# dphoyes/OpenCL-Structure-from-Motion

Measured on AMD Instinct MI355X. Metric: stereo frame-pairs/sec (1242x375) through pushBack+matchFeatures(2), p_matched bit-exact, higher is better.
Workload: dtype u8

## Files before the change

opencl-structure-from-motion_amd/csrc/vsm_dc.hip:

```cpp
#include <hip/hip_runtime.h>
#include <atomic>
#include <stdint.h>
#include <stdio.h>

#include <algorithm>
#include <mutex>
#include <vector>
#include <cmath>

#include "vsm_dc_gpu.h"
#include "vsm_dc_mesh.h"
#include "vsm_dc_lds.h"
#include "vsm_internal.h"

static const uint32_t *dc2_tiny_table();

#define KD_THREADS 1024
#define KD_CHUNKS 256
#define KD_DIGITS 128

__device__ inline uint32_t kd_block_scan(uint32_t v, uint32_t *tot) {
  const int lane = threadIdx.x & 63, wv = threadIdx.x >> 6;
  uint32_t x = v;
#pragma unroll
// ... 1224 lines not shown
      const int32_t div = nn[e] >> 1;
      if (q < off[e] + div) {
        nn[e] = div;
      } else {
        off[e] += div;
        nn[e] -= div;
      }
    }
    __syncthreads();
    if (cut_x) {
      uint16_t *w = Y;
      Y = Yn;
      Yn = w;
    } else {
      uint16_t *w = X;
      X = Xn;
      Xn = w;
    }
  }
  DC2_T(p4);
#pragma unroll
  for (int e = 0; e < E; e++) {
    const int q = E * t + e;
    if (q < m) jb.key[q] = jb.key_sorted[X[q]];
  }
#ifdef DC2_PHASE_TIMING
  if (t == 0) {
    const long long p5 = clock64();
    atomicAdd(&dc2_dbg[12][0], 1ull);
    DC2_ACC(12, 3, p2, p3);
    DC2_ACC(12, 4, p3, p4);
    DC2_ACC(12, 2, p4, p5);
  }
#endif
}

__device__ inline bool dc2_walk(int32_t m, int depth, uint32_t path, int32_t &off, int32_t &n, int &axis) {
  off = 0;
  n = m;
  axis = 0;
  for (int b = depth - 1; b >= 0; b--) {
    if (n <= VSM_DC_BLOCK_POINTS) return false;
    const int32_t div = n >> 1;
    if ((path >> b) & 1) {
      off += div;
      n -= div;
    } else {
      n = div;
    }
    axis = 1 - axis;
  }
  return true;
}

#define DC2_REACH_ALL 0x7fff8000u
#define DC2_REACH_NONE 0x80007fffu
__device__ inline uint32_t dc2_reach_word(double c, double rad) {
  const double lo = floor(c - rad), hi = ceil(c + rad);
  if (!(lo == lo) || !(hi == hi)) return DC2_REACH_ALL;
  const int32_t l = lo < -32768.0 ? -32768 : (lo > 32767.0 ? 32767 : (int32_t)lo);
  const int32_t h = hi > 32767.0 ? 32767 : (hi < -32768.0 ? -32768 : (int32_t)hi);
  return ((uint32_t)l & 0xffffu) | ((uint32_t)h << 16);
}
__device__ inline void dc2_reach(uint32_t pa, uint32_t pb, uint32_t pc, uint32_t &wx, uint32_t &wy) {
  const double ax = (double)(pa & 0xffffu), ay = (double)(pa >> 16);
  const double bx = (double)(pb & 0xffffu) - ax, by = (double)(pb >> 16) - ay;
  const double cx = (double)(pc & 0xffffu) - ax, cy = (double)(pc >> 16) - ay;
  const double d = 2.0 * (bx * cy - by * cx);
  const double b2 = bx * bx + by * by, c2 = cx * cx + cy * cy;
  const double ux = (cy * b2 - by * c2) / d, uy = (bx * c2 - cx * b2) / d;
  const double rad = sqrt(ux * ux + uy * uy) + 1.5;
  if (!(d == d) || d == 0.0 || !(rad == rad)) {
    wx = wy = DC2_REACH_ALL;
    return;
  }
  wx = dc2_reach_word(ax + ux, rad);
  wy = dc2_reach_word(ay + uy, rad);
}
__device__ inline bool dc2_reaches(uint32_t w, bool left_half, int32_t cl, int32_t cr) {
  const int32_t lo = (int32_t)(int16_t)(w & 0xffffu), hi = (int32_t)(int16_t)(w >> 16);
  return left_half ? hi >= cr : lo <= cl;
}

#ifndef DC2_BLOCK_WAVES
#define DC2_BLOCK_WAVES 4
#endif
#define DC2_BLOCK_THREADS (64 * DC2_BLOCK_WAVES)
#ifndef DC2_BLOCK_PACKED
#define DC2_BLOCK_PACKED 16
#endif
#ifndef DC2_BLOCK_OCC
#define DC2_BLOCK_OCC 5
#endif
#ifndef DC2_BLOCK_TAIL
#if defined(__gfx900__) || defined(__gfx906__) || defined(__gfx908__) || defined(__gfx90a__) || defined(__gfx940__) || defined(__gfx941__) || \
    defined(__gfx942__) || defined(__gfx950__) || !defined(__HIP_DEVICE_COMPILE__)
#define DC2_BLOCK_TAIL 1
#else
#define DC2_BLOCK_TAIL DC2_BLOCK_WAVES
#endif
#endif
__global__ void __launch_bounds__(DC2_BLOCK_THREADS, DC2_BLOCK_OCC) k_dc2_block(const VsmDc2Job *__restrict__ jobs, int depth) {
  __shared__ __attribute__((aligned(16))) uint32_t s_w[2 * VSM_DC_BLOCK_POINTS * 4];
  __shared__ uint32_t s_pt[VSM_DC_BLOCK_POINTS];
  __shared__ Dc2Hull16 s_hull[2 << DC2_BLOCK_DEPTH];
  const VsmDc2Job j2 = jobs[blockIdx.y];
  const int32_t m = j2.mn[0];
  if (m < 2) return;
  int32_t boff = 0, bn = m;
  int baxis = 0, d = 0;
  uint32_t bidx = 1;
  const uint32_t path = blockIdx.x;
  for (int b = depth - 1; b >= 0 && bn > VSM_DC_BLOCK_POINTS; b--, d++) {
    const int32_t div = bn >> 1;
    if ((path >> b) & 1) {
      boff += div;
      bn -= div;
      bidx = 2 * bidx + 1;
    } else {
      bn = div;
      bidx = 2 * bidx;
    }
    baxis = 1 - baxis;
  }
  if (bn > VSM_DC_BLOCK_POINTS) {
    if (threadIdx.x == 0) *j2.error = 2;
    return;
  }
  if (d < depth && (path & ((1u << (depth - d)) - 1u)) != 0) return;
  const int lane = threadIdx.x;
  const int wv = lane >> 6, wl = lane & 63;
  DC2_T(c0);
  {
    dc2_v4u ones;
    ones.x = ones.y = ones.z = ones.w = 0xffffffffu;
    for (int i = lane; i < 2 * bn; i += DC2_BLOCK_THREADS) ((dc2_v4u *)s_w)[i] = ones;
  }
  __syncthreads();
  DcBlockMesh mesh;
  mesh.w = (DC2_AS3 dc2_u32a *)s_w;
  mesh.pt = (DC2_AS3 const uint32_t *)s_pt;
  mesh.key = j2.key + boff;
  mesh.ptw = (DC2_AS3 uint32_t *)s_pt;
  mesh.gid = j2.id + boff;
  DC2_T(c1);
  {
    constexpr int kPerWave = (1 << DC2_BLOCK_DEPTH) / DC2_BLOCK_WAVES;
    for (int v = wl; v < kPerWave; v += 64) dc2_block_leaf_run(mesh, wv * kPerWave + v, bn, baxis, (DC2_AS3 Dc2Hull16 *)s_hull);
  }
  __syncthreads();
  DC2_T(c2);
#ifdef DC2_PHASE_TIMING
  long long cl = c2;
#endif
  for (int L = DC2_BLOCK_DEPTH - 1; L >= 0; L--) {
    {
      const int nodes = 1 << L;
      int node = -1;
      if (nodes >= DC2_BLOCK_PACKED) {
        if (DC2_BLOCK_TAIL < DC2_BLOCK_WAVES && wv >= DC2_BLOCK_TAIL && wv * 64 >= nodes) return;
        node = lane < nodes ? lane : -1;
      } else if (nodes >= DC2_BLOCK_TAIL) {
        const int per_wave = nodes / DC2_BLOCK_TAIL;
        if (wv >= DC2_BLOCK_TAIL) return;
        node = wl < per_wave ? wv * per_wave + wl : -1;
      } else {
        if (wv >= nodes && DC2_BLOCK_TAIL < DC2_BLOCK_WAVES) return;
        node = wl == 0 && wv < nodes ? wv : -1;
      }
      if (node >= 0) dc2_block_merge_run(mesh, node, L, bn, baxis, (DC2_AS3 Dc2Hull16 *)s_hull);
    }
    __syncthreads();
#ifdef DC2_PHASE_TIMING
    {
      const long long cn = clock64();
      if (lane == 0) DC2_ACC(0, 3 + L, cl, cn);
      cl = cn;
    }
#endif
  }
  DC2_T(c3);
  dc2_v4i *gt = (dc2_v4i *)(j2.tri + (size_t)2 * boff * 8);
  constexpr int kLive = DC2_BLOCK_TAIL < DC2_BLOCK_WAVES ? 64 : DC2_BLOCK_THREADS;
  for (int t = lane; t < 2 * bn; t += kLive) {
    const dc2_v4u o = ((const dc2_v4u *)s_w)[t];
    auto nb = [&](uint32_t v) -> int32_t { return (v & 0xffffu) == 0xffffu ? -1 : (int32_t)(v & 0xffffu) + 8 * boff; };
    auto vx = [&](uint32_t v) -> int32_t { return (v >> 16) == 0xffffu ? -1 : (int32_t)(v >> 16) + boff; };
    dc2_v4i a, b;
    a.x = nb(o.x);
    a.y = nb(o.y);
    a.z = nb(o.z);
    b.x = vx(o.x);
    b.y = vx(o.y);
    b.z = vx(o.z);
    uint32_t wx, wy;
    if ((b.x & b.y & b.z) < 0)
      wx = wy = DC2_REACH_NONE;
    else if ((b.x | b.y | b.z) < 0)
      wx = wy = DC2_REACH_ALL;
    else
      dc2_reach(s_pt[o.x >> 16], s_pt[o.y >> 16], s_pt[o.z >> 16], wx, wy);
    a.w = (int32_t)wy;
    b.w = (int32_t)wx;
    gt[2 * t] = a;
    gt[2 * t + 1] = b;
  }
  for (int i = lane; i < bn; i += kLive) j2.pt[boff + i] = s_pt[i];
  if (lane == 0) {
    const Dc2Hull16 hl = s_hull[1];
    j2.hulls[bidx] = VsmDcHull{hl.fl_t + 2 * boff, hl.fl_o, hl.fr_t + 2 * boff, hl.fr_o};
  }
#ifdef DC2_PHASE_TIMING
  if (lane == 0) {
    const long long c4 = clock64();
    atomicAdd(&dc2_dbg[0][0], 1ull);
    DC2_ACC(0, 1, c0, c1);
    DC2_ACC(0, 2, c1, c2);
    DC2_ACC(0, 13, c3, c4);
    DC2_ACC(0, 14, c0, c4);
  }
#endif
}

#ifndef DC2_MERGE_THREADS
#define DC2_MERGE_THREADS 256
#endif
#ifndef DC2_BAND_BATCH
#define DC2_BAND_BATCH 8
#endif
#ifdef DC2_PHASE_TIMING
#define DC2_BAND_STAT(level, col, v) atomicAdd(&dc2_dbg[1 + (level)][col], (unsigned long long)(v))
#else
#define DC2_BAND_STAT(level, col, v)
#endif

__device__ inline uint32_t dc2_mask_prefix(const uint32_t *mask, uint16_t *pre, int words, uint32_t *tot) {
  const int t = threadIdx.x, lane = t & 63, wv = t >> 6;
  const int per = (words + DC2_MERGE_THREADS - 1) / DC2_MERGE_THREADS;
  const int w0 = min(words, t * per), w1 = min(words, w0 + per);
  uint32_t sum = 0;
  for (int w = w0; w < w1; w++) sum += __popc(mask[w]);
  uint32_t x = sum;
#pragma unroll
  for (int d = 1; d < 64; d <<= 1) {
    const uint32_t y = __shfl_up(x, d, 64);
    if (lane >= d) x += y;
  }
  if (lane == 63) tot[wv] = x;
  __syncthreads();
  uint32_t base = 0, total = 0;
  for (int k = 0; k < DC2_MERGE_THREADS / 64; k++) {
    base += k < wv ? tot[k] : 0u;
    total += tot[k];
  }
  uint32_t run = base + x - sum;
  for (int w = w0; w < w1; w++) {
    pre[w] = (uint16_t)run;
    run += __popc(mask[w]);
  }
  __syncthreads();
  return total;
}
__device__ inline bool dc2_bit(const uint32_t *mask, int i) { return (mask[i >> 5] >> (i & 31)) & 1u; }
__device__ inline int dc2_rank(const uint32_t *mask, const uint16_t *pre, int i) {
  return (int)pre[i >> 5] + __popc(mask[i >> 5] & ((1u << (i & 31)) - 1u));
}

__global__ void __launch_bounds__(DC2_MERGE_THREADS) k_dc2_merge(const VsmDc2Job *__restrict__ jobs, int level, int lines_cap, int pts_cap, int words_cap) {
  extern __shared__ __attribute__((aligned(16))) uint8_t dc2_lds[];
  uint16_t *s_rec = (uint16_t *)dc2_lds;
  uint32_t *s_pt = (uint32_t *)(s_rec + (size_t)lines_cap * 8);
  uint32_t *s_l2s = s_pt + pts_cap;
  uint32_t *s_c2p = s_l2s + lines_cap;
  uint32_t *s_band = s_c2p + pts_cap;
  uint32_t *s_ring = s_band + words_cap;
  uint32_t *s_pmask = s_ring + words_cap;
  uint16_t *s_bpre = (uint16_t *)(s_pmask + (words_cap + 1) / 2);
  uint16_t *s_ppre = s_bpre + words_cap;
  __shared__ int32_t s_cl, s_cr, s_fail;
  __shared__ uint32_t s_tot[DC2_MERGE_THREADS / 64];
  const VsmDc2Job jb = jobs[blockIdx.y];
  const int32_t m = jb.mn[0];
  if (m < 2) return;
  int32_t off, n;
  int axis;
  if (!dc2_walk(m, level, blockIdx.x, off, n, axis) || n <= VSM_DC_BLOCK_POINTS) return;
  const uint32_t idx = (1u << level) | blockIdx.x;
  const int t = threadIdx.x;
  const int32_t div = n >> 1;
  const VsmDcHull l = jb.hulls[2 * idx], r = jb.hulls[2 * idx + 1];
  const int32_t tbase = 2 * off, nslots = 2 * n, tbase4 = 4 * tbase;
  const int bwords = (nslots + 31) >> 5, pwords = (n + 31) >> 5;
  int32_t *gnode = jb.tri + (size_t)tbase * 8;
  const dc2_v4i *grec = (const dc2_v4i *)gnode;
  const uint32_t *gpt = jb.pt + off;
  DC2_T(m0);
  bool band_ok = bwords <= words_cap;
  if (t == 0) {
    s_cl = -1;
    s_cr = 1 << 30;
    s_fail = 0;
  }
  if (band_ok) {
    for (int i = t; i < bwords; i += DC2_MERGE_THREADS) {
      s_band[i] = 0;
      s_ring[i] = 0;
    }
    for (int i = t; i < pwords; i += DC2_MERGE_THREADS) s_pmask[i] = 0;
    __syncthreads();
    {
      int32_t cl = -1, cr = 1 << 30;
      for (int i0 = t; i0 < n; i0 += DC2_BAND_BATCH * DC2_MERGE_THREADS) {
        uint32_t p[DC2_BAND_BATCH];
#pragma unroll
        for (int k = 0; k < DC2_BAND_BATCH; k++) {
          const int i = i0 + k * DC2_MERGE_THREADS;
          p[k] = i < n ? gpt[i] : 0u;
        }
#pragma unroll
        for (int k = 0; k < DC2_BAND_BATCH; k++) {
          const int i = i0 + k * DC2_MERGE_THREADS;
          const int32_t c = axis == 0 ? (int32_t)(p[k] & 0xffffu) : (int32_t)(p[k] >> 16);
          if (i < div)
            cl = max(cl, c);
          else if (i < n)
            cr = min(cr, c);
        }
      }
#pragma unroll
      for (int o = 32; o >= 1; o >>= 1) {
        cl = max(cl, __shfl_xor(cl, o, 64));
        cr = min(cr, __shfl_xor(cr, o, 64));
      }
      if ((t & 63) == 0) {
        atomicMax(&s_cl, cl);
        atomicMin(&s_cr, cr);
      }
    }
    __syncthreads();
    const int32_t cl = s_cl, cr = s_cr;
    {
      const int32_t *gw = gnode + (axis == 0 ? 7 : 3);
      for (int s0 = t; s0 < nslots; s0 += DC2_BAND_BATCH * DC2_MERGE_THREADS) {
        uint32_t w[DC2_BAND_BATCH];
#pragma unroll
        for (int k = 0; k < DC2_BAND_BATCH; k++) {
          const int s = s0 + k * DC2_MERGE_THREADS;
          w[k] = s < nslots ? (uint32_t)gw[(size_t)s * 8] : DC2_REACH_NONE;
        }
#pragma unroll
        for (int k = 0; k < DC2_BAND_BATCH; k++) {
          const int s = s0 + k * DC2_MERGE_THREADS;
          const bool hot = s < nslots && (s == 2 * div - 2 || s == 2 * div - 1 || dc2_reaches(w[k], s < 2 * div, cl, cr));
          if (hot) atomicOr(&s_band[s >> 5], 1u << (s & 31));
        }
      }
    }
    __syncthreads();
    const int s_own = 2 * div - 2;
    for (int s0 = t; s0 < nslots; s0 += DC2_BAND_BATCH * DC2_MERGE_THREADS) {
      dc2_v4i e[DC2_BAND_BATCH];
      bool hot[DC2_BAND_BATCH];
#pragma unroll
      for (int k = 0; k < DC2_BAND_BATCH; k++) {
        const int s = s0 + k * DC2_MERGE_THREADS;
        hot[k] = s < nslots && dc2_bit(s_band, s);
        e[k] = grec[2 * (hot[k] ? s : s_own)];
      }
#pragma unroll
      for (int k = 0; k < DC2_BAND_BATCH; k++) {
        if (!hot[k]) continue;
        const int32_t nb[3] = {e[k].x, e[k].y, e[k].z};
#pragma unroll
        for (int o = 0; o < 3; o++) {
          if (nb[o] < 0) continue;
          const int s2 = (nb[o] - tbase4) >> 2;
          if (s2 >= 0 && s2 < nslots) atomicOr(&s_ring[s2 >> 5], 1u << (s2 & 31));
        }
      }
    }
    __syncthreads();
    for (int i = t; i < bwords; i += DC2_MERGE_THREADS) s_band[i] |= s_ring[i];
    __syncthreads();
    const uint32_t nlines = dc2_mask_prefix(s_band, s_bpre, bwords, s_tot);
    uint32_t npts = 0;
    band_ok = nlines + 1 <= (uint32_t)lines_cap;
    if (band_ok) {
      for (int s = t; s < nslots; s += DC2_MERGE_THREADS)
        if (dc2_bit(s_band, s)) s_l2s[dc2_rank(s_band, s_bpre, s)] = (uint32_t)s;
      __syncthreads();
      for (uint32_t k0 = t; k0 < nlines; k0 += 3 * DC2_MERGE_THREADS) {
        dc2_v4i v[3];
#pragma unroll
        for (int k = 0; k < 3; k++) {
          const uint32_t ln = k0 + k * DC2_MERGE_THREADS;
          v[k] = grec[2 * (ln < nlines ? (int)s_l2s[ln] : s_own) + 1];
        }
#pragma unroll
        for (int k = 0; k < 3; k++) {
          if (k0 + k * DC2_MERGE_THREADS >= nlines) continue;
          const int32_t vv[3] = {v[k].x, v[k].y, v[k].z};
#pragma unroll
          for (int o = 0; o < 3; o++)
            if (vv[o] >= 0) atomicOr(&s_pmask[(vv[o] - off) >> 5], 1u << ((vv[o] - off) & 31));
        }
      }
      __syncthreads();
      npts = dc2_mask_prefix(s_pmask, s_ppre, pwords, s_tot);
      band_ok = npts <= (uint32_t)pts_cap;
      if (band_ok) {
        for (int i0 = t; i0 < n; i0 += DC2_BAND_BATCH * DC2_MERGE_THREADS) {
          uint32_t p[DC2_BAND_BATCH];
#pragma unroll
          for (int k = 0; k < DC2_BAND_BATCH; k++) {
            const int i = i0 + k * DC2_MERGE_THREADS;
            p[k] = gpt[i < n ? i : 0];
          }
#pragma unroll
          for (int k = 0; k < DC2_BAND_BATCH; k++) {
            const int i = i0 + k * DC2_MERGE_THREADS;
            if (i < n && dc2_bit(s_pmask, i)) {
              const int c = dc2_rank(s_pmask, s_ppre, i);
              s_pt[c] = p[k];
              s_c2p[c] = (uint32_t)i;
            }
          }
        }
        for (uint32_t k0 = t; k0 < nlines; k0 += 3 * DC2_MERGE_THREADS) {
          dc2_v4i e3[3], v3[3];
#pragma unroll
          for (int k = 0; k < 3; k++) {
            const uint32_t ln = k0 + k * DC2_MERGE_THREADS;
            const int s = ln < nlines ? (int)s_l2s[ln] : s_own;
            e3[k] = grec[2 * s];
            v3[k] = grec[2 * s + 1];
          }
#pragma unroll
          for (int k = 0; k < 3; k++) {
            const uint32_t line = k0 + k * DC2_MERGE_THREADS;
            if (line >= nlines) continue;
            const dc2_v4i e = e3[k], v = v3[k];
            auto nbw = [&](int32_t g) -> uint32_t {
              if (g < 0) return 4 * nlines;
              const int s2 = (g - tbase4) >> 2;
              if (s2 < 0 || s2 >= nslots || !dc2_bit(s_band, s2)) return 4 * nlines;
              return (uint32_t)(dc2_rank(s_band, s_bpre, s2) * 4 + (g & 3));
            };
            auto vxw = [&](int32_t g) -> uint32_t { return g < 0 ? 0xffffu : (uint32_t)dc2_rank(s_pmask, s_ppre, g - off); };
            dc2_v4u o;
            o.x = nbw(e.x) | (vxw(v.x) << 16);
            o.y = nbw(e.y) | (vxw(v.y) << 16);
            o.z = nbw(e.z) | (vxw(v.z) << 16);
            o.w = 0xffffffffu;
            ((dc2_v4u *)s_rec)[line] = o;
          }
        }
      }
    }
    __syncthreads();
    DC2_T(m1);
    if (band_ok) {
      if (t == 0) {
        DcBandMesh mesh;
        mesh.w = (DC2_AS3 dc2_u32a *)s_rec;
        mesh.pt = (DC2_AS3 const uint32_t *)s_pt;
        mesh.rim = 4 * (int32_t)nlines;
        mesh.budget = 8 * (int32_t)nlines + 64;
        mesh.make_trap();
        auto ln = [&](int32_t gt) -> int32_t {
          if (!dc2_bit(s_band, gt - tbase)) mesh.tripped = 1;
          return dc2_rank(s_band, s_bpre, gt - tbase);
        };
        DcOTri fl{ln(l.fl_t), l.fl_o}, il{ln(l.fr_t), l.fr_o}, ir{ln(r.fl_t), r.fl_o}, fr{ln(r.fr_t), r.fr_o};
        int32_t tcur = dc2_rank(s_band, s_bpre, 2 * div - 2);
        if (mesh.ok()) dc_merge(mesh, fl, il, ir, fr, axis, tcur);
        if (mesh.ok() && !mesh.trap_touched())
          jb.hulls[idx] = VsmDcHull{(int32_t)s_l2s[fl.t] + tbase, fl.o, (int32_t)s_l2s[fr.t] + tbase, fr.o};
        else
          s_fail = 1;
      }
      __syncthreads();
      band_ok = s_fail == 0;
#ifdef DC2_PHASE_TIMING
      if (t == 0) {
        const long long m2 = clock64();
        atomicAdd(&dc2_dbg[1 + level][0], 1ull);
        DC2_ACC(1 + level, 1, m0, m1);
        DC2_ACC(1 + level, 2, m1, m2);
        DC2_BAND_STAT(level, 3, nlines);
        DC2_BAND_STAT(level, 4, band_ok ? 0 : 1);
        atomicMax(&dc2_dbg[1 + level][6], (unsigned long long)nlines);
        atomicMax(&dc2_dbg[1 + level][7], (unsigned long long)npts);
      }
#endif
      if (band_ok) {
        for (uint32_t k = t; k < nlines; k += DC2_MERGE_THREADS) {
          const dc2_v4u o = ((const dc2_v4u *)s_rec)[k];
          auto nb = [&](uint32_t v) -> int32_t { return v == 0xffffu ? -1 : (int32_t)(s_l2s[v >> 2] * 4 + (v & 3)) + tbase4; };
          auto vx = [&](uint32_t v) -> int32_t { return v == 0xffffu ? -1 : (int32_t)s_c2p[v] + off; };
          const uint32_t rimh = 4 * nlines;
          const int32_t s = (int32_t)s_l2s[k];
          const dc2_v4i old = grec[2 * s];
          dc2_v4i a, b;
          a.x = (o.x & 0xffffu) == rimh ? old.x : nb(o.x & 0xffffu);
          a.y = (o.y & 0xffffu) == rimh ? old.y : nb(o.y & 0xffffu);
          a.z = (o.z & 0xffffu) == rimh ? old.z : nb(o.z & 0xffffu);
          b.x = vx(o.x >> 16);
          b.y = vx(o.y >> 16);
          b.z = vx(o.z >> 16);
          uint32_t wx, wy;
          if ((b.x & b.y & b.z) < 0)
            wx = wy = DC2_REACH_NONE;
          else if ((b.x | b.y | b.z) < 0)
            wx = wy = DC2_REACH_ALL;
          else
            dc2_reach(s_pt[o.x >> 16], s_pt[o.y >> 16], s_pt[o.z >> 16], wx, wy);
          a.w = (int32_t)wy;
          b.w = (int32_t)wx;
          ((dc2_v4i *)gnode)[2 * s] = a;
          ((dc2_v4i *)gnode)[2 * s + 1] = b;
        }
        return;
      }
    }
  }
  if (t == 0) {
    DcOTri fl{l.fl_t, l.fl_o}, il{l.fr_t, l.fr_o}, ir{r.fl_t, r.fl_o}, fr{r.fr_t, r.fr_o};
    int32_t tg = 2 * (off + div) - 2;
    const DcMesh mesh{jb.tri, jb.pt, jb.id, jb.key};
    mesh.merge_hulls(fl, il, ir, fr, axis, tg);
    jb.hulls[idx] = VsmDcHull{fl.t, fl.o, fr.t, fr.o};
#ifdef DC2_PHASE_TIMING
    atomicAdd(&dc2_dbg[1 + level][5], 1ull);
#endif
  }
  __threadfence();
  __syncthreads();
  for (int sl = t; sl < nslots; sl += DC2_MERGE_THREADS) {
    const int32_t vx0 = __hip_atomic_load(gnode + (size_t)sl * 8 + 4, __ATOMIC_RELAXED, __HIP_MEMORY_SCOPE_AGENT);
    const int32_t vx1 = __hip_atomic_load(gnode + (size_t)sl * 8 + 5, __ATOMIC_RELAXED, __HIP_MEMORY_SCOPE_AGENT);
    const int32_t vx2 = __hip_atomic_load(gnode + (size_t)sl * 8 + 6, __ATOMIC_RELAXED, __HIP_MEMORY_SCOPE_AGENT);
    uint32_t wx, wy;
    if ((vx0 & vx1 & vx2) < 0)
      wx = wy = DC2_REACH_NONE;
    else if ((vx0 | vx1 | vx2) < 0)
      wx = wy = DC2_REACH_ALL;
    else
      dc2_reach(jb.pt[vx0], jb.pt[vx1], jb.pt[vx2], wx, wy);
    gnode[(size_t)sl * 8 + 3] = (int32_t)wy;
    gnode[(size_t)sl * 8 + 7] = (int32_t)wx;
  }
}

template <int CAP>
__global__ void __launch_bounds__(64) k_dc2_ties(const VsmDc2Job *__restrict__ jobs, int32_t *__restrict__ tie_out, int out_stride, const uint32_t *__restrict__ tiny) {
  const VsmDc2Job jb = jobs[blockIdx.x];
  int32_t *out = tie_out ? tie_out + (size_t)blockIdx.x * out_stride : const_cast<int32_t *>(jb.tie_out);
  const int n = *jb.count;
  if (n <= 3 || n > jb.cap) {
    if (threadIdx.x == 0) out[0] = n <= 3 ? 0 : -1;
    return;
  }
  tie_sort<CAP>(TieFromKeys{jb.keys_in}, n, out, tiny);
}

__global__ void __launch_bounds__(64) k_dc2_apply_ties(const VsmDc2Job *__restrict__ jobs) {
  const VsmDc2Job jb = jobs[blockIdx.x];
  const int32_t c = jb.tie_out[0];
  if (c < 0) {
    if (threadIdx.x == 0 && jb.mn[0] >= 2) *jb.error = 3;
    return;
  }
  for (int k = threadIdx.x; k < c; k += 64) {
    const int32_t rep = jb.tie_out[1 + 2 * k], first = jb.tie_out[2 + 2 * k];
    if (rep >= 0 && rep < jb.cap) jb.remap[rep] = first;
  }
}

__global__ void __launch_bounds__(256) k_dc2_flows(const VsmDc2Job *__restrict__ jobs, int method) {
  const VsmDc2Job jb = jobs[blockIdx.y];
  const int n = jb.mn[1];
  const int i = blockIdx.x * blockDim.x + threadIdx.x;
  if (i >= n || jb.mn[0] < 2) return;
  const vsm_p_match a = jb.list[i];
  float *fu = (float *)jb.kd_scratch, *fv = fu + jb.kd_stride, *dp = fv + jb.kd_stride;
  fu[i] = a.u1c - a.u1p;
  fv[i] = a.v1c - a.v1p;
  dp[i] = method == 1 ? a.u1c - a.u2c : a.u1p - a.u2p;
}

__global__ void __launch_bounds__(256) k_dc2_support(const VsmDc2Job *__restrict__ jobs, int method, float ftol, float dtol) {
  const VsmDc2Job jb = jobs[blockIdx.y];
  const int32_t m = jb.mn[0];
  const int t = blockIdx.x * blockDim.x + threadIdx.x;
  if (m < 2 || t >= 2 * m) return;
  const int4 v = *(const int4 *)(jb.tri + (size_t)t * 8 + 4);
  if ((v.x | v.y | v.z) < 0) return;
  const int32_t q[3] = {jb.remap[jb.id[v.y]], jb.remap[jb.id[v.z]], jb.remap[jb.id[v.x]]};
  const float *fua = (const float *)jb.kd_scratch, *fva = fua + jb.kd_stride, *dpa = fva + jb.kd_stride;
  float fu[3], fv[3], dp[3];
#pragma unroll
  for (int k = 0; k < 3; k++) {
    fu[k] = fua[q[k]];
    fv[k] = fva[q[k]];
    dp[k] = dpa[q[k]];
  }
#pragma unroll
  for (int e = 0; e < 3; e++) {
// ... 334 lines not shown
```

opencl-structure-from-motion_amd/csrc/vsm_seq2.inc:

```
#include "vsm_dc_gpu.h"

struct Dc2Bank {
  int npairs = 0, cap = 0;
  bool host_ties = false;
  uint8_t *d_block = nullptr, *h_block = nullptr, *h_block_dev = nullptr;
  VsmDc2Job *h_jobs = nullptr, *d_jobs = nullptr;
  int32_t *d_ties = nullptr;
  uint64_t *h_keys = nullptr;
  int32_t *h_n = nullptr, *h_ties = nullptr, *h_error = nullptr;
  int ties_stride = 0;
  size_t pair_stride = 0;
  struct PairPtr {
    uint64_t *keys_in, *key_sorted, *key;
    uint32_t *kd, *pt;
    int32_t *id, *tri, *mn, *support, *remap, *out_count;
    VsmDcHull *hulls;
  };
  std::vector<PairPtr> pp;
  void release() {
    if (d_block) vsm_dev_free(d_block);
    if (h_block) (void)hipHostFree(h_block);
    if (h_jobs) (void)hipHostFree(h_jobs);
    *this = Dc2Bank();
  }
  static size_t al(size_t x) { return (x + 255) & ~(size_t)255; }
  bool reserve(int pairs, int want_cap, bool with_host_ties) {
    if (pairs <= npairs && want_cap <= cap && (!with_host_ties || host_ties)) return true;
    const int ncap = std::max(((want_cap + 1023) / 1024) * 1024, cap), np = std::max(pairs, npairs);
    const bool ht = with_host_ties || host_ties;
    release();
    npairs = np;
    cap = ncap;
    host_ties = ht;
    const size_t c = (size_t)cap;
    const size_t per = al(c * 8) * 3 + al(c * 4 * VSM_DC_KD_SCRATCH) + al(c * 4) * 4 + al(c * 64) + al(64) +
                       al(sizeof(VsmDcHull) * (2u << VSM_DC2_MAX_DEPTH));
    pair_stride = per;
    const size_t d_bytes = per * npairs + al(sizeof(VsmDc2Job) * npairs) + al((size_t)npairs * VSM_DC_TIE_OUT_INTS * 4);
    ties_stride = cap + 2;
    const size_t h_bytes = al(64) + (ht ? (al(c * 8) + al((size_t)ties_stride * 4)) * npairs : 0) + al((size_t)npairs * 4);
    if (vsm_dev_alloc((void **)&d_block, d_bytes) != hipSuccess || hipHostMalloc((void **)&h_block, h_bytes, hipHostMallocMapped) != hipSuccess ||
        hipHostGetDevicePointer((void **)&h_block_dev, h_block, 0) != hipSuccess ||
        hipHostMalloc((void **)&h_jobs, sizeof(VsmDc2Job) * npairs, hipHostMallocDefault) != hipSuccess) {
      release();
      return false;
    }
    memset(h_block, 0, h_bytes);
    pp.resize(npairs);
    uint8_t *b = d_block;
    auto take = [&](size_t bytes) {
      uint8_t *r = b;
      b += al(bytes);
      return r;
    };
    for (int i = 0; i < npairs; i++) {
      PairPtr &q = pp[i];
      q.keys_in = (uint64_t *)take(c * 8);
      q.key_sorted = (uint64_t *)take(c * 8);
      q.key = (uint64_t *)take(c * 8);
      q.kd = (uint32_t *)take(c * 4 * VSM_DC_KD_SCRATCH);
      q.pt = (uint32_t *)take(c * 4);
      q.id = (int32_t *)take(c * 4);
      q.support = (int32_t *)take(c * 4);
      q.remap = (int32_t *)take(c * 4);
      q.tri = (int32_t *)take(c * 64);
      q.mn = (int32_t *)take(64);
      q.out_count = q.mn + 4;
      q.hulls = (VsmDcHull *)take(sizeof(VsmDcHull) * (2u << VSM_DC2_MAX_DEPTH));
    }
    d_jobs = (VsmDc2Job *)take(sizeof(VsmDc2Job) * npairs);
    d_ties = (int32_t *)take((size_t)npairs * VSM_DC_TIE_OUT_INTS * 4);
    size_t ho = 0;
    h_error = (int32_t *)(h_block + ho);
    ho += al(64);
    h_n = (int32_t *)(h_block + ho);
    ho += al((size_t)npairs * 4);
    if (ht) {
      h_keys = (uint64_t *)(h_block + ho);
      ho += al(c * 8) * npairs;
      h_ties = (int32_t *)(h_block + ho);
    }
    return true;
  }
  uint64_t *host_keys(int i) const { return (uint64_t *)((uint8_t *)h_keys + al((size_t)cap * 8) * i); }
  int32_t *host_ties_of(int i) const { return (int32_t *)((uint8_t *)h_ties + al((size_t)ties_stride * 4) * i); }
  template <typename T>
  T *dev_of(T *host_ptr) const {
    return (T *)(h_block_dev + ((uint8_t *)host_ptr - h_block));
  }
  void fill_job(int i, const vsm_p_match *list, const int32_t *count, bool gpu_ties, vsm_p_match *out, int32_t *h_out_count,
                float *ranges, uint32_t *h_keep = nullptr, bool keys_by_dma = false) {
    const PairPtr &q = pp[i];
    VsmDc2Job &jb = h_jobs[i];
    memset(&jb, 0, sizeof(jb));
    jb.list = list;
    jb.count = count;
    jb.cap = cap;
    jb.kd_stride = cap;
    jb.keys_in = q.keys_in;
    jb.h_keys = (!gpu_ties && host_ties && !keys_by_dma) ? dev_of(host_keys(i)) : nullptr;
    jb.h_n = dev_of(h_n + i);
    jb.key_sorted = q.key_sorted;
    jb.key = q.key;
    jb.kd_scratch = q.kd;
    jb.pt = q.pt;
    jb.id = q.id;
    jb.tri = q.tri;
    jb.hulls = q.hulls;
    jb.mn = q.mn;
    jb.support = q.support;
// ... 746 lines not shown
      for (int j = 0; j < k; j++) {
        const int rc = finish_chain1_of(j);
        if (rc != VSM_OK) return rc;
      }
    const double t0 = now_us();
    HIPCHK(hipEventSynchronize(h->seq_ev[0]));
    HIPCHK(hipGetLastError());
    tg += now_us() - t0;
    dbg_counts.push_back(now_us());
    q.max_nq[0] = q.max_nq[1] = 0;
    q.valid = std::make_shared<std::vector<char>>(n, 0);
    for (int i = 0; i < n; i++) {
      const int32_t f = q.f0 + i;
      VsmJob &jb = h_jobs[i];
      memset(&jb, 0, sizeof(jb));
      const int img_c = first_img + sides * i;
      int img_p;
      int32_t cnt[4][2];
      for (int s = 0; s < 2; s++) {
        cnt[2][s] = c.hm_counts[img_c * 2 + s];
        cnt[3][s] = right ? c.hm_counts[(img_c + 1) * 2 + s] : 0;
      }
      if (method == 1) {
        img_p = img_c;
        for (int s = 0; s < 2; s++) cnt[0][s] = cnt[1][s] = 0;
      } else if (i > 0) {
        img_p = img_c - sides;
        for (int s = 0; s < 2; s++) {
          cnt[0][s] = c.hm_counts[img_p * 2 + s];
          cnt[1][s] = right ? c.hm_counts[(img_p + 1) * 2 + s] : 0;
        }
      } else {
        img_p = sides * ((k + kFrameBanks - 1) % kFrameBanks) * C + sides * ((k > 0 ? chunk_start[k] - chunk_start[k - 1] : 1) - 1);
        for (int s = 0; s < 2; s++) {
          cnt[0][s] = f > 0 ? nprev[0][s] : 0;
          cnt[1][s] = f > 0 ? nprev[1][s] : 0;
        }
      }
      jb.img_prev = img_p;
      jb.img_curr = img_c;
      if (match_ready(p, method, cnt)) {
        (*q.valid)[i] = 1;
        const int qimg = method == 2 ? 0 : 2;
        jb.nq[0] = p.multi_stage ? cnt[qimg][0] : 0;
        jb.nq[1] = cnt[qimg][1];
        if (Tr && (!Tr_valid || Tr_valid[f])) {
          jb.use_tr = 1;
          memcpy(jb.t, Tr + (size_t)f * 12, 12 * sizeof(double));
        }
      }
      q.max_nq[0] = std::max(q.max_nq[0], jb.nq[0]);
      q.max_nq[1] = std::max(q.max_nq[1], jb.nq[1]);
    }
    for (int s = 0; s < 2; s++) {
      nprev[0][s] = c.hm_counts[(first_img + sides * (n - 1)) * 2 + s];
      nprev[1][s] = right ? c.hm_counts[(first_img + sides * (n - 1) + 1) * 2 + s] : 0;
    }
    if (q.max_nq[0] > VSM_DC_TIE_POINTS || q.max_nq[1] > VSM_DC_KD_MAX_POINTS || (p.refinement == 2 && q.max_nq[1] > VSM_PARA_MAX_LIST) ||
        vsm_dc2_depth(std::max(q.max_nq[0], q.max_nq[1])) > VSM_DC2_MAX_DEPTH) {
      declined = true;
      return VSM_OK;
    }
    HIPCHK(vsm_upload(h->stream, d_jobs, h_jobs, sizeof(VsmJob) * n));
    if (p.multi_stage) {
      VsmMatchCfg cfg = make_cfg(p, method, h->sw.match_heads && c.has_heads);
      VsmJob dummy;
      memset(&dummy, 0, sizeof(dummy));
      cfg.sparse = 1;
      cfg.use_prior = 0;
      vsm_launch_match(h->stream, h->prof, c.d_imgs, d_pairs, d_jobs, dummy, n, c.dims, cfg, q.max_nq[0]);
      q.ev_p1 = S.get_event();
      q.ev_prior = S.get_event();
      if (!q.ev_p1 || !q.ev_prior) return VSM_EHIP;
      HIPCHK(hipEventRecord(q.ev_p1, h->stream));
    }
    return VSM_OK;
  };
  auto start_chain1 = [&](int k) -> int {
    Ck &q = ck[k];
    if (!p.multi_stage) return VSM_OK;
    const int n = q.n, first_pair = q.first_pair;
    {
      Dc2Bank &B = S.bank1[k & 1];
      if (!B.reserve(C, std::max(q.max_nq[0], 64), ties1_host)) return VSM_EHIP;
      if (S.bank1_copied[k & 1]) HIPCHK(hipEventSynchronize(S.bank1_copied[k & 1]));
      for (int i = 0; i < n; i++)
        B.fill_job(i, c.h_pairs[first_pair + i].list1, c.h_pairs[first_pair + i].count, !ties1_host, nullptr, nullptr,
                   c.h_pairs[first_pair + i].ranges);
      hipStream_t c1 = S.cs(k);
      if (k > 1 && ck[k - 2].ev_prior) HIPCHK(hipStreamWaitEvent(c1, ck[k - 2].ev_prior, 0));
      HIPCHK(hipStreamWaitEvent(c1, q.ev_p1, 0));
      HIPCHK(vsm_upload(c1, B.d_jobs, B.h_jobs, sizeof(VsmDc2Job) * n));
      S.bank1_copied[k & 1] = S.get_event();
      if (!S.bank1_copied[k & 1]) return VSM_EHIP;
      HIPCHK(hipEventRecord(S.bank1_copied[k & 1], c1));
      h->prof.begin(VSM_K_DC_KEYS, c1);
      vsm_dc2_launch_keys(c1, B.d_jobs, n, q.max_nq[0]);
      h->prof.end(c1);
      hipEvent_t ev_keys = S.get_event(), ev_ties = S.get_event();
      if (!ev_keys || !ev_ties) return VSM_EHIP;
      HIPCHK(hipEventRecord(ev_keys, c1));
      if (ties1_host) {
        q.ev_k1 = ev_keys;
        q.chain1_open = true;
        dc2_enqueue_mesh(c1, B, n, q.max_nq[0], h->prof, false, nullptr, S.expect_long);
        HIPCHK(hipGetLastError());
        return VSM_OK;
      }
      hipStream_t ts1 = inorder ? h->stream : (sw.seq_ties1_null ? S.ns : S.cs(k + 2));
      HIPCHK(hipStreamWaitEvent(ts1, ev_keys, 0));
      h->prof.begin(VSM_K_DC_TIES, ts1);
      vsm_dc2_launch_ties(ts1, B.d_jobs, n, B.d_ties, VSM_DC_TIE_OUT_INTS, q.max_nq[0]);
      h->prof.end(ts1);
      HIPCHK(hipEventRecord(ev_ties, ts1));
      dc2_enqueue_mesh(c1, B, n, q.max_nq[0], h->prof, false, nullptr, S.expect_long);
      HIPCHK(hipStreamWaitEvent(c1, ev_ties, 0));
      dc2_enqueue_votes(c1, B, n, q.max_nq[0], method, (float)p.outlier_flow_tolerance, (float)p.outlier_disp_tolerance, h->prof);
      h->prof.begin(VSM_K_DC_PRIOR, c1);
      vsm_dc2_launch_prior(c1, B.d_jobs, n, method, p.match_binsize, p.match_radius, w, hh, c.dims.ub, c.dims.vb);
      h->prof.end(c1);
      HIPCHK(hipGetLastError());
      HIPCHK(hipEventRecord(q.ev_prior, c1));
    }
    return VSM_OK;
  };
  auto finish_chain1 = [&](int k) -> int {
    Ck &q = ck[k];
    if (!q.chain1_open) return VSM_OK;
    q.chain1_open = false;
    Dc2Bank &B = S.bank1[k & 1];
    const int n = q.n;
    const double t0 = now_us();
    HIPCHK(hipEventSynchronize(q.ev_k1));
    h->pool->run(n, [&](int i) {
      static thread_local ExactDelaunay sorter;
      const int32_t nl = B.h_n[i];
      int32_t *out = B.host_ties_of(i);
      out[0] = (nl > 3 && nl <= B.cap) ? sorter.sort_ties(B.host_keys(i), nl, out + 1, (B.ties_stride - 1) / 2) : 0;
    });
    tg += now_us() - t0;
    hipStream_t c1 = S.cs(k);
    std::lock_guard<std::mutex> lk(S.enq_mu);
    dc2_enqueue_votes(c1, B, n, q.max_nq[0], method, (float)p.outlier_flow_tolerance, (float)p.outlier_disp_tolerance, h->prof);
    h->prof.begin(VSM_K_DC_PRIOR, c1);
    vsm_dc2_launch_prior(c1, B.d_jobs, n, method, p.match_binsize, p.match_radius, w, hh, c.dims.ub, c.dims.vb);
    h->prof.end(c1);
    HIPCHK(hipGetLastError());
    HIPCHK(hipEventRecord(q.ev_prior, c1));
    return VSM_OK;
  };
  finish_chain1_of = finish_chain1;
  auto launch_refine = [&](Seq2Chunk *ch, int k) -> int {
    const Ck &q = ck[k];
    VsmJob dummy;
    memset(&dummy, 0, sizeof(dummy));
    if (p.refinement > 0)
      vsm_launch_refine(h->stream, h->prof, c.d_imgs, c.d_pairs + q.first_pair, c.d_jobs + q.first_pair, dummy, q.n, c.dims, c.dims, method,
                        p.refinement, q.max_nq[1]);
    if (p.refinement == 2) vsm_launch_parabolic_apply(h->stream, c.d_pairs + q.first_pair, q.n);
    ch->ev_ref = S.get_event();
    if (!ch->ev_ref) return VSM_EHIP;
    HIPCHK(hipEventRecord(ch->ev_ref, h->stream));
    return VSM_OK;
  };
  int exp_k = 0;
  auto export_some = [&](int upto, int budget) -> int {
// ... 465 lines not shown
```

Measured before the change: 54230.

## Track per-node boundary-crossing triangle lists to shrink merge band discovery

Leaf blocks and merge kernels now record each node's point bounding box and a compact list of triangles whose circumcircle reach crosses that box. Parent merges seed the band from these candidate lists instead of scanning all slots and points to find the seam band. Point compaction is also rewritten to iterate set mask bits. The host now waits for the prior chunk before a bank reallocation, which guards against freeing memory still in use. This adds atomics, extra global writes and scratch-space use, and falls back to the full scan when a list overflows.

```diff
diff --git a/opencl-structure-from-motion_amd/csrc/vsm_dc.hip b/opencl-structure-from-motion_amd/csrc/vsm_dc.hip
--- a/opencl-structure-from-motion_amd/csrc/vsm_dc.hip
+++ b/opencl-structure-from-motion_amd/csrc/vsm_dc.hip
@@ -1330,6 +1330,17 @@
   return left_half ? hi >= cr : lo <= cl;
 }
 
+static_assert(VSM_DC_KD_SCRATCH >= 7, "node summaries: arrays 3..6, beside the flows' 0..2");
+__device__ inline uint32_t *dc2_sum_list(const VsmDc2Job &jb, int level) { return jb.kd_scratch + (size_t)(3 + (level & 1)) * jb.kd_stride; }
+__device__ inline uint4 *dc2_sum_meta(const VsmDc2Job &jb) { return (uint4 *)(jb.kd_scratch + (size_t)5 * jb.kd_stride); }
+__device__ inline bool dc2_crosses(uint32_t wx, uint32_t wy, uint32_t bx, uint32_t by) {
+  return (int32_t)(int16_t)(wx & 0xffffu) <= (int32_t)(bx & 0xffffu) || (int32_t)(int16_t)(wx >> 16) >= (int32_t)(bx >> 16) ||
+         (int32_t)(int16_t)(wy & 0xffffu) <= (int32_t)(by & 0xffffu) || (int32_t)(int16_t)(wy >> 16) >= (int32_t)(by >> 16);
+}
+__device__ inline uint32_t dc2_box_union(uint32_t a, uint32_t b) {
+  return min(a & 0xffffu, b & 0xffffu) | (max(a >> 16, b >> 16) << 16);
+}
+
 #ifndef DC2_BLOCK_WAVES
 #define DC2_BLOCK_WAVES 4
 #endif
@@ -1352,6 +1363,7 @@
   __shared__ __attribute__((aligned(16))) uint32_t s_w[2 * VSM_DC_BLOCK_POINTS * 4];
   __shared__ uint32_t s_pt[VSM_DC_BLOCK_POINTS];
   __shared__ Dc2Hull16 s_hull[2 << DC2_BLOCK_DEPTH];
+  __shared__ uint32_t s_box[4], s_cnt;
   const VsmDc2Job j2 = jobs[blockIdx.y];
   const int32_t m = j2.mn[0];
   if (m < 2) return;
@@ -1379,6 +1391,11 @@
   const int lane = threadIdx.x;
   const int wv = lane >> 6, wl = lane & 63;
   DC2_T(c0);
+  if (lane == 0) {
+    s_box[0] = s_box[2] = 0xffffu;
+    s_box[1] = s_box[3] = 0u;
+    s_cnt = 0u;
+  }
   {
     dc2_v4u ones;
     ones.x = ones.y = ones.z = ones.w = 0xffffffffu;
@@ -1428,8 +1445,34 @@
 #endif
   }
   DC2_T(c3);
+  constexpr int kLive = DC2_BLOCK_TAIL < DC2_BLOCK_WAVES ? 64 : DC2_BLOCK_THREADS;
+  {
+    uint32_t x0 = 0xffffu, x1 = 0u, y0 = 0xffffu, y1 = 0u;
+    for (int i = lane; i < bn; i += kLive) {
+      const uint32_t p = s_pt[i];
+      x0 = min(x0, p & 0xffffu);
+      x1 = max(x1, p & 0xffffu);
+      y0 = min(y0, p >> 16);
+      y1 = max(y1, p >> 16);
+    }
+#pragma unroll
+    for (int o = 32; o >= 1; o >>= 1) {
+      x0 = min(x0, (uint32_t)__shfl_xor((int)x0, o, 64));
+      x1 = max(x1, (uint32_t)__shfl_xor((int)x1, o, 64));
+      y0 = min(y0, (uint32_t)__shfl_xor((int)y0, o, 64));
+      y1 = max(y1, (uint32_t)__shfl_xor((int)y1, o, 64));
+    }
+    if (wl == 0) {
+      atomicMin(&s_box[0], x0);
+      atomicMax(&s_box[1], x1);
+      atomicMin(&s_box[2], y0);
+      atomicMax(&s_box[3], y1);
+    }
+  }
+  __syncthreads();
+  const uint32_t box_x = s_box[0] | s_box[1] << 16, box_y = s_box[2] | s_box[3] << 16;
+  uint32_t *slist = dc2_sum_list(j2, d) + boff;
   dc2_v4i *gt = (dc2_v4i *)(j2.tri + (size_t)2 * boff * 8);
-  constexpr int kLive = DC2_BLOCK_TAIL < DC2_BLOCK_WAVES ? 64 : DC2_BLOCK_THREADS;
   for (int t = lane; t < 2 * bn; t += kLive) {
     const dc2_v4u o = ((const dc2_v4u *)s_w)[t];
     auto nb = [&](uint32_t v) -> int32_t { return (v & 0xffffu) == 0xffffu ? -1 : (int32_t)(v & 0xffffu) + 8 * boff; };
@@ -1452,11 +1495,17 @@
     b.w = (int32_t)wx;
     gt[2 * t] = a;
     gt[2 * t + 1] = b;
+    if (dc2_crosses(wx, wy, box_x, box_y)) {
+      const uint32_t k = atomicAdd(&s_cnt, 1u);
+      if (k < (uint32_t)bn) slist[k] = (uint32_t)(2 * boff + t);
+    }
   }
   for (int i = lane; i < bn; i += kLive) j2.pt[boff + i] = s_pt[i];
+  __syncthreads();
   if (lane == 0) {
     const Dc2Hull16 hl = s_hull[1];
     j2.hulls[bidx] = VsmDcHull{hl.fl_t + 2 * boff, hl.fl_o, hl.fr_t + 2 * boff, hl.fr_o};
+    dc2_sum_meta(j2)[bidx] = make_uint4(box_x, box_y, s_cnt <= (uint32_t)bn ? s_cnt : 0xffffffffu, 0u);
   }
 #ifdef DC2_PHASE_TIMING
   if (lane == 0) {
@@ -1526,7 +1575,7 @@
   uint16_t *s_bpre = (uint16_t *)(s_pmask + (words_cap + 1) / 2);
   uint16_t *s_ppre = s_bpre + words_cap;
   __shared__ int32_t s_cl, s_cr, s_fail;
-  __shared__ uint32_t s_tot[DC2_MERGE_THREADS / 64];
+  __shared__ uint32_t s_tot[DC2_MERGE_THREADS / 64], s_cnt;
   const VsmDc2Job jb = jobs[blockIdx.y];
   const int32_t m = jb.mn[0];
   if (m < 2) return;
@@ -1542,12 +1591,23 @@
   int32_t *gnode = jb.tri + (size_t)tbase * 8;
   const dc2_v4i *grec = (const dc2_v4i *)gnode;
   const uint32_t *gpt = jb.pt + off;
+  uint4 *meta = dc2_sum_meta(jb);
+  const uint4 ml = meta[2 * idx], mr = meta[2 * idx + 1];
+  const uint32_t box_x = dc2_box_union(ml.x, mr.x), box_y = dc2_box_union(ml.y, mr.y);
+  const int32_t ecl = (int32_t)((axis == 0 ? ml.x : ml.y) >> 16), ecr = (int32_t)((axis == 0 ? mr.x : mr.y) & 0xffffu);
+  const int32_t nl = (int32_t)ml.z, nr = (int32_t)mr.z;
+  const bool lists = nl >= 0 && nl <= div && nr >= 0 && nr <= n - div && ecl <= ecr;
+  const uint32_t *listl = dc2_sum_list(jb, level + 1) + off, *listr = listl + div;
+  const int ncand = lists ? nl + nr : 0;
+  uint32_t *slist = dc2_sum_list(jb, level) + off;
+  auto cand = [&](int k) -> int { return (int)(k < nl ? listl[k] : listr[k - nl]) - tbase; };
   DC2_T(m0);
   bool band_ok = bwords <= words_cap;
   if (t == 0) {
     s_cl = -1;
     s_cr = 1 << 30;
     s_fail = 0;
+    s_cnt = 0;
   }
   if (band_ok) {
     for (int i = t; i < bwords; i += DC2_MERGE_THREADS) {
@@ -1556,6 +1616,26 @@
     }
     for (int i = t; i < pwords; i += DC2_MERGE_THREADS) s_pmask[i] = 0;
     __syncthreads();
+  }
+  const int s_own = 2 * div - 2;
+  if (band_ok && lists) {
+    for (int k = t; k < ncand + 2; k += DC2_MERGE_THREADS) {
+      const int s = k < ncand ? cand(k) : s_own + (k - ncand);
+      if (s < 0 || s >= nslots) continue;
+      const bool hot = k >= ncand || dc2_reaches((uint32_t)gnode[(size_t)s * 8 + (axis == 0 ? 7 : 3)], s < 2 * div, ecl, ecr);
+      if (!hot) continue;
+      atomicOr(&s_band[s >> 5], 1u << (s & 31));
+      const dc2_v4i e = grec[2 * s];
+      const int32_t nb[3] = {e.x, e.y, e.z};
+#pragma unroll
+      for (int o = 0; o < 3; o++) {
+        if (nb[o] < 0) continue;
+        const int s2 = (nb[o] - tbase4) >> 2;
+        if (s2 >= 0 && s2 < nslots) atomicOr(&s_ring[s2 >> 5], 1u << (s2 & 31));
+      }
+    }
+    __syncthreads();
+  } else if (band_ok) {
     {
       int32_t cl = -1, cr = 1 << 30;
       for (int i0 = t; i0 < n; i0 += DC2_BAND_BATCH * DC2_MERGE_THREADS) {
@@ -1605,7 +1685,6 @@
       }
     }
     __syncthreads();
-    const int s_own = 2 * div - 2;
     for (int s0 = t; s0 < nslots; s0 += DC2_BAND_BATCH * DC2_MERGE_THREADS) {
       dc2_v4i e[DC2_BAND_BATCH];
       bool hot[DC2_BAND_BATCH];
@@ -1628,6 +1707,8 @@
       }
     }
     __syncthreads();
+  }
+  if (band_ok) {
     for (int i = t; i < bwords; i += DC2_MERGE_THREADS) s_band[i] |= s_ring[i];
     __syncthreads();
     const uint32_t nlines = dc2_mask_prefix(s_band, s_bpre, bwords, s_tot);
@@ -1657,23 +1738,16 @@
       npts = dc2_mask_prefix(s_pmask, s_ppre, pwords, s_tot);
       band_ok = npts <= (uint32_t)pts_cap;
       if (band_ok) {
-        for (int i0 = t; i0 < n; i0 += DC2_BAND_BATCH * DC2_MERGE_THREADS) {
-          uint32_t p[DC2_BAND_BATCH];
-#pragma unroll
-          for (int k = 0; k < DC2_BAND_BATCH; k++) {
-            const int i = i0 + k * DC2_MERGE_THREADS;
-            p[k] = gpt[i < n ? i : 0];
-          }
-#pragma unroll
-          for (int k = 0; k < DC2_BAND_BATCH; k++) {
-            const int i = i0 + k * DC2_MERGE_THREADS;
-            if (i < n && dc2_bit(s_pmask, i)) {
-              const int c = dc2_rank(s_pmask, s_ppre, i);
-              s_pt[c] = p[k];
-              s_c2p[c] = (uint32_t)i;
-            }
+        for (int w = t; w < pwords; w += DC2_MERGE_THREADS) {
+          uint32_t bits = s_pmask[w];
+          uint32_t c = s_ppre[w];
+          while (bits) {
+            s_c2p[c++] = (uint32_t)(w * 32 + __ffs(bits) - 1);
+            bits &= bits - 1u;
           }
         }
+        __syncthreads();
+        for (uint32_t c = t; c < npts; c += DC2_MERGE_THREADS) s_pt[c] = gpt[s_c2p[c]];
         for (uint32_t k0 = t; k0 < nlines; k0 += 3 * DC2_MERGE_THREADS) {
           dc2_v4i e3[3], v3[3];
 #pragma unroll
@@ -1767,11 +1841,28 @@
           b.w = (int32_t)wx;
           ((dc2_v4i *)gnode)[2 * s] = a;
           ((dc2_v4i *)gnode)[2 * s + 1] = b;
+          if (lists && dc2_crosses(wx, wy, box_x, box_y)) {
+            const uint32_t q = atomicAdd(&s_cnt, 1u);
+            if (q < (uint32_t)n) slist[q] = (uint32_t)(s + tbase);
+          }
         }
+        if (lists) {
+          for (int k = t; k < ncand; k += DC2_MERGE_THREADS) {
+            const int s = cand(k);
+            if (s < 0 || s >= nslots || dc2_bit(s_band, s)) continue;
+            if (dc2_crosses((uint32_t)gnode[(size_t)s * 8 + 7], (uint32_t)gnode[(size_t)s * 8 + 3], box_x, box_y)) {
+              const uint32_t q = atomicAdd(&s_cnt, 1u);
+              if (q < (uint32_t)n) slist[q] = (uint32_t)(s + tbase);
+            }
+          }
+        }
+        __syncthreads();
+        if (t == 0) meta[idx] = make_uint4(box_x, box_y, lists && s_cnt <= (uint32_t)n ? s_cnt : 0xffffffffu, 0u);
         return;
       }
     }
   }
+  if (t == 0) meta[idx] = make_uint4(box_x, box_y, 0xffffffffu, 0u);
   if (t == 0) {
     DcOTri fl{l.fl_t, l.fl_o}, il{l.fr_t, l.fr_o}, ir{r.fl_t, r.fl_o}, fr{r.fr_t, r.fr_o};
     int32_t tg = 2 * (off + div) - 2;
diff --git a/opencl-structure-from-motion_amd/csrc/vsm_seq2.inc b/opencl-structure-from-motion_amd/csrc/vsm_seq2.inc
--- a/opencl-structure-from-motion_amd/csrc/vsm_seq2.inc
+++ b/opencl-structure-from-motion_amd/csrc/vsm_seq2.inc
@@ -24,8 +24,11 @@
     *this = Dc2Bank();
   }
   static size_t al(size_t x) { return (x + 255) & ~(size_t)255; }
+  bool covers(int pairs, int want_cap, bool with_host_ties) const {
+    return pairs <= npairs && want_cap <= cap && (!with_host_ties || host_ties);
+  }
   bool reserve(int pairs, int want_cap, bool with_host_ties) {
-    if (pairs <= npairs && want_cap <= cap && (!with_host_ties || host_ties)) return true;
+    if (covers(pairs, want_cap, with_host_ties)) return true;
     const int ncap = std::max(((want_cap + 1023) / 1024) * 1024, cap), np = std::max(pairs, npairs);
     const bool ht = with_host_ties || host_ties;
     release();
@@ -938,6 +941,8 @@
     const int n = q.n, first_pair = q.first_pair;
     {
       Dc2Bank &B = S.bank1[k & 1];
+      if (!B.covers(C, std::max(q.max_nq[0], 64), ties1_host) && k > 1 && ck[k - 2].ev_prior)
+        HIPCHK(hipEventSynchronize(ck[k - 2].ev_prior));
       if (!B.reserve(C, std::max(q.max_nq[0], 64), ties1_host)) return VSM_EHIP;
       if (S.bank1_copied[k & 1]) HIPCHK(hipEventSynchronize(S.bank1_copied[k & 1]));
       for (int i = 0; i < n; i++)
```

After: 54720, median of 6. No clear change (+0.9%).
